# quartiq/stabilizer-stream

Measured on NVIDIA B200. Metric: sustained MS/s through full PSD cascade, higher is better.
Workload: dtype f32

## Files before the change

### stabilizer_stream_b200/csrc/sspsd_cascade.cu

```cuda
#if defined(__x86_64__)
#include <emmintrin.h>
#endif

#include "sspsd_cascade.cuh"

#include <algorithm>
#include <cmath>
#include <cstdlib>
#include <cstring>
#include <mutex>

#include "sspsd_decim_kernel.cuh"
#include "sspsd_stage_kernel.cuh"
#include "sspsd_stage_kernel_r16.cuh"
#include "sspsd_stage_kernel_ring.cuh"
#include "sspsd_stage_kernel_w16.cuh"

namespace sspsd {

static thread_local std::string g_err;
void set_error(const std::string& msg) { g_err = msg; }
const char* last_error() { return g_err.c_str(); }

bool cuda_ok(cudaError_t e, const char* what)
// ... 78 lines not shown
        SSPSD_CUDA(cudaFuncSetAttribute(psd_stage_kernel_ring1x5, cudaFuncAttributeMaxDynamicSharedMemorySize,
                                        (int)stage_ring_smem_bytes(384, 1, 3, false)));
        return SSPSD_OK;
    }
    if (log2n == 9)
        SSPSD_CUDA(cudaFuncSetAttribute(psd_stage_kernel_w16, cudaFuncAttributeMaxDynamicSharedMemorySize,
                                        (int)stage_w16_smem_bytes(W16::MAX_T)));
    switch (log2n) {
#define X(L)                                                                   \
    case L:                                                                    \
        *nt = Plan<L>::NT;                                                     \
        return prepare_stage_t<L>(hop, Plan<L>::NT <= 256 ? 100 * 1024 : 200 * 1024, tmax);
        SSPSD_FOR_SIZES(X)
#undef X
    default:
        set_error("n_fft must be a power of two in 64..8192");
        return SSPSD_EINVAL;
    }
}

template <int MA, int MB, int MC, int PRESET>
int launch_decim_t(const DecimParams& p, int grid, cudaStream_t s)
{
    using GE = DecGeom<MA, MB, MC>;
    decim8_kernel<MA, MB, MC, PRESET><<<grid, DEC_NT, GE::SMEM_FLOATS * sizeof(float), s>>>(p);
    return cuda_ok(cudaGetLastError(), "decim8_kernel launch") ? SSPSD_OK : SSPSD_ECUDA;
}

template <int MA, int MB, int MC, int PRESET, int OB, int CTAS>
int launch_decim_tma_t(const DecimParams& p, long long n_out, int num_sms, cudaStream_t s)
{
    const int ntiles = (int)((n_out + OB - 1) / OB);
    const int grid = std::min(ntiles, num_sms * CTAS);
    decim8_tma_kernel<MA, MB, MC, PRESET, OB, CTAS><<<grid, DEC_NT, decim_tma_smem_bytes<MA, MB, MC, OB>(), s>>>(p, ntiles);
    return cuda_ok(cudaGetLastError(), "decim8_tma_kernel launch") ? SSPSD_OK : SSPSD_ECUDA;
}

template <int MA, int MB, int MC, int PRESET, int OB, int CTAS>
int launch_decim_async_t(const DecimParams& p, long long n_out, int num_sms, cudaStream_t s)
{
    const int ntiles = (int)((n_out + OB - 1) / OB);
    const int grid = std::min(ntiles, num_sms * CTAS);
    decim8_async_kernel<MA, MB, MC, PRESET, OB, CTAS><<<grid, DEC_NT, decim_async_smem_bytes<MA, MB, MC, OB>(), s>>>(p, ntiles);
    return cuda_ok(cudaGetLastError(), "decim8_async_kernel launch") ? SSPSD_OK : SSPSD_ECUDA;
}

template <int MA, int MB, int MC, int PRESET, int OB, int CTAS>
int launch_decim_pf_t(const DecimParams& p, long long n_out, int num_sms, cudaStream_t s)
{
    const int ntiles = (int)((n_out + OB - 1) / OB);
    const int grid = std::min(ntiles, num_sms * CTAS);
    decim8_pf_kernel<MA, MB, MC, PRESET, OB, CTAS><<<grid, DEC_NT, decim_pf_smem_bytes<MA, MB, MC, OB>(), s>>>(p, ntiles);
    return cuda_ok(cudaGetLastError(), "decim8_pf_kernel launch") ? SSPSD_OK : SSPSD_ECUDA;
}

int decim_halo(int preset)
{
    return preset == SSPSD_HBF_98 ? DecGeom<3, 6, 15>::HALO : DecGeom<5, 10, 23>::HALO;
}

int upload_taps_once(int device)
{
    static std::mutex mu;
    static bool done[64] = {false};
    std::lock_guard<std::mutex> lock(mu);
    if (device < 64 && done[device])
        return SSPSD_OK;
    static_assert(sizeof(sspsd_hbf_taps) == sizeof(float) * SSPSD_HBF_NPRESET * 3 * SSPSD_HBF_MAXTAPS, "tap table");
    {
        float t0[SSPSD_HBF_NPRESET][3][SSPSD_HBF_MAXTAPS + 1], t1[SSPSD_HBF_NPRESET][3][SSPSD_HBF_MAXTAPS + 1];
        for (int p = 0; p < SSPSD_HBF_NPRESET; ++p)
            for (int s = 0; s < 3; ++s)
                for (int i = 0; i <= SSPSD_HBF_MAXTAPS; ++i) {
                    t0[p][s][i] = i < SSPSD_HBF_MAXTAPS ? sspsd_hbf_taps[p][s][i] : 0.f;
                    t1[p][s][i] = i + 1 < SSPSD_HBF_MAXTAPS ? sspsd_hbf_taps[p][s][i + 1] : 0.f;
                }
        SSPSD_CUDA(cudaMemcpyToSymbol(c_hbf_taps, t0, sizeof(t0)));
        SSPSD_CUDA(cudaMemcpyToSymbol(c_hbf_taps_sh, t1, sizeof(t1)));
    }
    SSPSD_CUDA(cudaFuncSetAttribute(decim8_kernel<5, 10, 23, SSPSD_HBF_140>, cudaFuncAttributeMaxDynamicSharedMemorySize,
                                    (int)(DecGeom<5, 10, 23>::SMEM_FLOATS * sizeof(float))));
    SSPSD_CUDA(cudaFuncSetAttribute(decim8_kernel<3, 6, 15, SSPSD_HBF_98>, cudaFuncAttributeMaxDynamicSharedMemorySize,
                                    (int)(DecGeom<3, 6, 15>::SMEM_FLOATS * sizeof(float))));
    SSPSD_CUDA(cudaFuncSetAttribute(decim8_async_kernel<5, 10, 23, SSPSD_HBF_140, 960, 2>,
                                    cudaFuncAttributeMaxDynamicSharedMemorySize, (int)decim_async_smem_bytes<5, 10, 23, 960>()));
    SSPSD_CUDA(cudaFuncSetAttribute(decim8_async_kernel<5, 10, 23, SSPSD_HBF_140, 640, 3>,
                                    cudaFuncAttributeMaxDynamicSharedMemorySize, (int)decim_async_smem_bytes<5, 10, 23, 640>()));
    SSPSD_CUDA(cudaFuncSetAttribute(decim8_async_kernel<3, 6, 15, SSPSD_HBF_98, 960, 2>,
                                    cudaFuncAttributeMaxDynamicSharedMemorySize, (int)decim_async_smem_bytes<3, 6, 15, 960>()));
    SSPSD_CUDA(cudaFuncSetAttribute(decim8_async_kernel<3, 6, 15, SSPSD_HBF_98, 640, 3>,
                                    cudaFuncAttributeMaxDynamicSharedMemorySize, (int)decim_async_smem_bytes<3, 6, 15, 640>()));
    SSPSD_CUDA(cudaFuncSetAttribute(decim8_tma_kernel<5, 10, 23, SSPSD_HBF_140, 960, 2>,
                                    cudaFuncAttributeMaxDynamicSharedMemorySize, (int)decim_tma_smem_bytes<5, 10, 23, 960>()));
    SSPSD_CUDA(cudaFuncSetAttribute(decim8_tma_kernel<5, 10, 23, SSPSD_HBF_140, 640, 3>,
                                    cudaFuncAttributeMaxDynamicSharedMemorySize, (int)decim_tma_smem_bytes<5, 10, 23, 640>()));
    SSPSD_CUDA(cudaFuncSetAttribute(decim8_tma_kernel<3, 6, 15, SSPSD_HBF_98, 960, 2>,
                                    cudaFuncAttributeMaxDynamicSharedMemorySize, (int)decim_tma_smem_bytes<3, 6, 15, 960>()));
    SSPSD_CUDA(cudaFuncSetAttribute(decim8_tma_kernel<3, 6, 15, SSPSD_HBF_98, 640, 3>,
                                    cudaFuncAttributeMaxDynamicSharedMemorySize, (int)decim_tma_smem_bytes<3, 6, 15, 640>()));
    SSPSD_CUDA(cudaFuncSetAttribute(decim8_tma_kernel<5, 10, 23, SSPSD_HBF_140, 768, 3>,
                                    cudaFuncAttributeMaxDynamicSharedMemorySize, (int)decim_tma_smem_bytes<5, 10, 23, 768>()));
    SSPSD_CUDA(cudaFuncSetAttribute(decim8_tma_kernel<3, 6, 15, SSPSD_HBF_98, 768, 3>,
                                    cudaFuncAttributeMaxDynamicSharedMemorySize, (int)decim_tma_smem_bytes<3, 6, 15, 768>()));
    SSPSD_CUDA(cudaFuncSetAttribute(decim8_pf_kernel<5, 10, 23, SSPSD_HBF_140, 960, 2>,
                                    cudaFuncAttributeMaxDynamicSharedMemorySize, (int)decim_pf_smem_bytes<5, 10, 23, 960>()));
    SSPSD_CUDA(cudaFuncSetAttribute(decim8_pf_kernel<5, 10, 23, SSPSD_HBF_140, 640, 3>,
                                    cudaFuncAttributeMaxDynamicSharedMemorySize, (int)decim_pf_smem_bytes<5, 10, 23, 640>()));
    SSPSD_CUDA(cudaFuncSetAttribute(decim8_pf_kernel<3, 6, 15, SSPSD_HBF_98, 960, 2>,
                                    cudaFuncAttributeMaxDynamicSharedMemorySize, (int)decim_pf_smem_bytes<3, 6, 15, 960>()));
    SSPSD_CUDA(cudaFuncSetAttribute(decim8_pf_kernel<3, 6, 15, SSPSD_HBF_98, 640, 3>,
                                    cudaFuncAttributeMaxDynamicSharedMemorySize, (int)decim_pf_smem_bytes<3, 6, 15, 640>()));
    if (device < 64)
        done[device] = true;
    return SSPSD_OK;
}

EwmaPlan ewma_plan(uint32_t count, uint32_t avg, uint64_t S)
{
    EwmaPlan e{};
    uint32_t steady = avg + 1u;
    e.g_s = (float)avg / (float)steady;
    uint64_t jb;
    if (count > avg) {
        jb = 0;
        e.g_first = (float)avg / (float)count;
    } else {
        jb = (uint64_t)avg - count + 1;
        e.g_first = e.g_s;
    }
    if (jb >= S) {
        e.jb = (int)S;
        e.total = 1.0f;
        e.count_after = (uint32_t)(count + S);
    } else {
        e.jb = (int)jb;
        double t = (double)e.g_first;
        uint64_t n_s = S - 1 - jb;
        if (n_s > 0)
            t *= std::pow((double)e.g_s, (double)n_s);
        e.total = (float)t;
        e.count_after = steady;
    }
    return e;
}

}

int hbf_info(int hbf, uint32_t* drain, uint32_t* halo)
{
    if (hbf != SSPSD_HBF_98 && hbf != SSPSD_HBF_140) return SSPSD_EINVAL;
    if (drain) *drain = (uint32_t)sspsd_hbf_drain[hbf];
    if (halo) *halo = (uint32_t)decim_halo(hbf);
    return SSPSD_OK;
}

Cascade::~Cascade()
{
    if (n_ == 0)
        return;
    DeviceGuard g(cfg_.device);
    if (stream_)
        cudaStreamSynchronize(stream_);
    if (deep_stream_) cudaStreamSynchronize(deep_stream_);
    if (psd_stream_) cudaStreamSynchronize(psd_stream_);
// ... 65 lines not shown
    std::vector<float> win(n);
    if (cfg.window == SSPSD_WINDOW_RECT) {
        std::fill(win.begin(), win.end(), 1.0f);
        win_ = {1.0f, 1.0f, 0};
    } else {
        const float pi = 3.14159265358979323846f;
        float df = pi / (float)n;
        for (uint32_t i = 0; i < n; ++i) {
            float s = sinf(df * (float)i);
            win[i] = s * s;
        }
        win_ = {0.25f, 1.5f, n / 2};
    }
    hop_ = n - win_.overlap;
    drain_ = sspsd_hbf_drain[cfg.hbf];
    int halo = decim_halo(cfg.hbf);
    hb_ = std::max<int>((int)win_.overlap, halo);
    hb_ = (hb_ + 7) & ~7;

    SSPSD_CUDA(cudaDeviceGetAttribute(&num_sms_, cudaDevAttrMultiProcessorCount, cfg.device));
    if (cfg.stream) {
        stream_ = (cudaStream_t)cfg.stream;
    } else {
        SSPSD_CUDA(cudaStreamCreateWithFlags(&stream_, cudaStreamNonBlocking));
        own_stream_ = true;
    }
    SSPSD_CUDA(cudaStreamCreateWithFlags(&copy_stream_, cudaStreamNonBlocking));
    const char* ov = getenv("SSPSD_OVERLAP");
    deep_from_ = ov ? (size_t)atoi(ov) : 1;
    if (max_stages_ > 1 && deep_from_ > 0 && !one_stream_) {
        int lo_prio = 0, hi_prio = 0;
        SSPSD_CUDA(cudaDeviceGetStreamPriorityRange(&lo_prio, &hi_prio));
        SSPSD_CUDA(cudaStreamCreateWithPriority(&deep_stream_, cudaStreamNonBlocking, hi_prio));
        SSPSD_CUDA(cudaEventCreateWithFlags(&ev_stage0_, cudaEventDisableTiming));
        SSPSD_CUDA(cudaEventCreateWithFlags(&ev_deep_, cudaEventDisableTiming));
        const char* ps = getenv("SSPSD_PSD_STREAM");
        if (!ps || atoi(ps) != 0) {
            SSPSD_CUDA(cudaStreamCreateWithPriority(&psd_stream_, cudaStreamNonBlocking, hi_prio));
            SSPSD_CUDA(cudaEventCreateWithFlags(&ev_psd_join_, cudaEventDisableTiming));
        }
    }
    for (int i = 0; i < 2; ++i) {
        SSPSD_CUDA(cudaEventCreateWithFlags(&ev_copied_[i], cudaEventDisableTiming));
        SSPSD_CUDA(cudaEventCreateWithFlags(&ev_free_[i], cudaEventDisableTiming));
        SSPSD_CUDA(cudaEventCreateWithFlags(&ev_stage_[i], cudaEventDisableTiming));
    }
    int rc = upload_taps_once(cfg.device);
    if (rc) return rc;
    defer_ = cfg_.deep_defer ? cfg_.deep_defer : (1ull << 26);
    if (const char* e = getenv("SSPSD_DEFER")) defer_ = strtoull(e, nullptr, 0);
    k2_variant_ = k2_variant_from_env();
    {
        const char* e = getenv("SSPSD_K3");
        std::string m = e ? e : "tma960";
        k3_variant_ = m == "tiled" ? 0 : m == "tma960" ? 1 : m == "tma640" ? 2 : m == "async640" ? 4 : m == "pf960" ? 5 :
                      m == "pf640" ? 6 : m == "tma768" ? 7 : 3;
    }
    rc = prepare_stage((int)log2n_, k2_variant_ >= 1, (int)hop_, &tmax_, &nt_);
    if (rc) return rc;

    const uint32_t m = n / 2;
    std::vector<float2> twM(m), twN(m);
    for (uint32_t k = 0; k < m; ++k) {
        double a = -2.0 * M_PI * (double)k / (double)m;
        twM[k] = make_float2((float)std::cos(a), (float)std::sin(a));
        double b = -2.0 * M_PI * (double)k / (double)n;
        twN[k] = make_float2((float)std::cos(b), (float)std::sin(b));
    }
    acc_stride_ = (m + 1 + 63) & ~63u;
    SSPSD_CUDA(cudaMalloc(&d_win_, n * sizeof(float)));
    SSPSD_CUDA(cudaMalloc(&d_twM_, m * sizeof(float2)));
    SSPSD_CUDA(cudaMalloc(&d_twN_, m * sizeof(float2)));
    SSPSD_CUDA(cudaMalloc(&d_acc_, (size_t)SSPSD_MAX_STAGES * acc_stride_ * sizeof(float)));
    SSPSD_CUDA(cudaMemcpyAsync(d_win_, win.data(), n * sizeof(float), cudaMemcpyHostToDevice, stream_));
    SSPSD_CUDA(cudaMemcpyAsync(d_twM_, twM.data(), m * sizeof(float2), cudaMemcpyHostToDevice, stream_));
    SSPSD_CUDA(cudaMemcpyAsync(d_twN_, twN.data(), m * sizeof(float2), cudaMemcpyHostToDevice, stream_));
    SSPSD_CUDA(cudaMemsetAsync(d_acc_, 0, (size_t)SSPSD_MAX_STAGES * acc_stride_ * sizeof(float), stream_));
    SSPSD_CUDA(cudaMallocHost(&h_acc_, (size_t)SSPSD_MAX_STAGES * acc_stride_ * sizeof(float)));
    SSPSD_CUDA(cudaStreamSynchronize(stream_));
    stages_.reserve(SSPSD_MAX_STAGES);
    n_ = n;
    return SSPSD_OK;
}

uint32_t Cascade::stage_avg(size_t i) const
{
    unsigned sh = (unsigned)(SSPSD_DEPTH * i);
    uint32_t v = sh >= 32 ? 0u : (avg_.count >> sh);
    return std::min(v, avg_.limit);
}

int Cascade::add_stage()
{
    if (stages_.size() >= SSPSD_MAX_STAGES) {
        set_error("too many stages");
        return SSPSD_EINVAL;
    }
    StageState st;
    const size_t cap = (size_t)hb_ + n_ + 16;
    cudaStream_t ss = stage_stream(stages_.size());
    if (!spare_.empty()) {
        StageState old = spare_.back();
        spare_.pop_back();
        st.carry[0] = old.carry[0];
        st.carry[1] = old.carry[1];
        st.fresh[0] = old.fresh[0];
        st.fresh[1] = old.fresh[1];
        st.fresh_cap = old.fresh_cap;
        st.ev_read[0] = old.ev_read[0];
// ... 156 lines not shown
    rc = launch_stage((int)log2n_, k2_variant_ >= 1, p, grid, psd_stream(i));
    prof_end(psd_stream(i));
    if (rc) return rc;
    return reduce_partials(i, grid * groups, p);
}

int Cascade::prepare_partials(size_t i, int rows, StageParams* p)
{
    p->part = nullptr;
    p->part_stride = 0;
    if (!(cfg_.flags & SSPSD_FLAG_DETERMINISTIC)) return SSPSD_OK;
    const int which = psd_stream(i) == stream_ ? 0 : 1;
    const size_t need = (size_t)rows * acc_stride_;
    if (need > part_cap_[which]) {
        SSPSD_CUDA(cudaStreamSynchronize(psd_stream(i)));
        if (d_part_[which]) SSPSD_CUDA(cudaFree(d_part_[which]));
        d_part_[which] = nullptr;
        SSPSD_CUDA(cudaMalloc(&d_part_[which], need * sizeof(float)));
        part_cap_[which] = need;
    }
    p->part = d_part_[which];
    p->part_stride = (int)acc_stride_;
    return SSPSD_OK;
}

int Cascade::reduce_partials(size_t i, int rows, const StageParams& p)
{
    if (!p.part) return SSPSD_OK;
    const int nb = (int)(n_ / 2 + 1);
    prof_begin(SSPSD_PROF_OTHER, 0, psd_stream(i));
    reduce_partials_kernel<<<(nb + 127) / 128, 128, 0, psd_stream(i)>>>(p.acc, p.part, rows, p.part_stride, nb);
    prof_end(psd_stream(i));
    return cuda_ok(cudaGetLastError(), "reduce_partials_kernel launch") ? SSPSD_OK : SSPSD_ECUDA;
}

int Cascade::launch_decim(size_t i, const StreamSrc& src, uint64_t m0, uint64_t m1, float* out_fresh,
                          long long out_split, long long out_cap)
{
    DecimParams p{};
    p.src = src;
    p.m0 = (long long)m0;
    p.m1 = (long long)m1;
    p.drain = drain_;
    p.out_fresh = out_fresh;
    p.out_split = out_split;
    p.out_cap = out_cap;
    p.preset = cfg_.hbf;
    long long lo = std::max<long long>(p.m0, p.drain);
    if (p.m1 <= lo)
        return SSPSD_OK;
    int grid = (int)((p.m1 - lo + DEC_OB - 1) / DEC_OB);
    cudaStream_t ss = stage_stream(i);
    static const bool fuse_carry = !getenv("SSPSD_CARRY_KERNEL");
    if (cc_valid_ && fuse_carry && (k3_variant_ == 1 || k3_variant_ == 2 || k3_variant_ == 7)) {
        p.cc = cc_pending_;
        cc_valid_ = false;
    }
    prof_begin(i == 0 ? SSPSD_PROF_DECIM_STAGE0 : SSPSD_PROF_DECIM_DEEP, (uint64_t)(p.m1 - lo) * 8, ss);
    int rc;
    if (k3_variant_ == 0) {
        rc = cfg_.hbf == SSPSD_HBF_98 ? launch_decim_t<3, 6, 15, SSPSD_HBF_98>(p, grid, ss)
                                      : launch_decim_t<5, 10, 23, SSPSD_HBF_140>(p, grid, ss);
    } else if (k3_variant_ == 1) {
        rc = cfg_.hbf == SSPSD_HBF_98 ? launch_decim_tma_t<3, 6, 15, SSPSD_HBF_98, 960, 2>(p, p.m1 - lo, num_sms_, ss)
                                      : launch_decim_tma_t<5, 10, 23, SSPSD_HBF_140, 960, 2>(p, p.m1 - lo, num_sms_, ss);
    } else if (k3_variant_ == 2) {
        rc = cfg_.hbf == SSPSD_HBF_98 ? launch_decim_tma_t<3, 6, 15, SSPSD_HBF_98, 640, 3>(p, p.m1 - lo, num_sms_, ss)
                                      : launch_decim_tma_t<5, 10, 23, SSPSD_HBF_140, 640, 3>(p, p.m1 - lo, num_sms_, ss);
    } else if (k3_variant_ == 3) {
        rc = cfg_.hbf == SSPSD_HBF_98 ? launch_decim_async_t<3, 6, 15, SSPSD_HBF_98, 960, 2>(p, p.m1 - lo, num_sms_, ss)
                                      : launch_decim_async_t<5, 10, 23, SSPSD_HBF_140, 960, 2>(p, p.m1 - lo, num_sms_, ss);
    } else if (k3_variant_ == 7) {
        rc = cfg_.hbf == SSPSD_HBF_98 ? launch_decim_tma_t<3, 6, 15, SSPSD_HBF_98, 768, 3>(p, p.m1 - lo, num_sms_, ss)
                                      : launch_decim_tma_t<5, 10, 23, SSPSD_HBF_140, 768, 3>(p, p.m1 - lo, num_sms_, ss);
    } else if (k3_variant_ == 5) {
        rc = cfg_.hbf == SSPSD_HBF_98 ? launch_decim_pf_t<3, 6, 15, SSPSD_HBF_98, 960, 2>(p, p.m1 - lo, num_sms_, ss)
                                      : launch_decim_pf_t<5, 10, 23, SSPSD_HBF_140, 960, 2>(p, p.m1 - lo, num_sms_, ss);
    } else if (k3_variant_ == 6) {
        rc = cfg_.hbf == SSPSD_HBF_98 ? launch_decim_pf_t<3, 6, 15, SSPSD_HBF_98, 640, 3>(p, p.m1 - lo, num_sms_, ss)
                                      : launch_decim_pf_t<5, 10, 23, SSPSD_HBF_140, 640, 3>(p, p.m1 - lo, num_sms_, ss);
    } else {
        rc = cfg_.hbf == SSPSD_HBF_98 ? launch_decim_async_t<3, 6, 15, SSPSD_HBF_98, 640, 3>(p, p.m1 - lo, num_sms_, ss)
                                      : launch_decim_async_t<5, 10, 23, SSPSD_HBF_140, 640, 3>(p, p.m1 - lo, num_sms_, ss);
    }
    prof_end(ss);
    return rc;
}

int Cascade::run_stage(size_t i, const float* fresh, long long split, uint64_t n_new)
{
    StageState& st = stages_[i];
    cudaStream_t ss = stage_stream(i);
    cudaStream_t ps = psd_stream(i);
    const uint64_t L1 = st.L + n_new;
    const uint64_t craw0 = st.craw;
    const uint64_t craw1 = L1 < n_ ? 0 : 1 + (L1 - n_) / hop_;
    const StreamSrc src{st.carry[st.cur], fresh, st.carry_start, split, (long long)L1};
    int rc;
    bool psd_launched = false;
    if (ps != ss && craw1 > craw0) {
        SSPSD_CUDA(cudaEventRecord(st.ev_in, ss));
        SSPSD_CUDA(cudaStreamWaitEvent(ps, st.ev_in, 0));
    }

    if (windowed_ && i < n_local_ && craw1 > craw0) {
        const uint64_t step = (uint64_t)hop_ << (SSPSD_DEPTH * i);
        const uint64_t c = own_offset(i);
        auto first_at_or_after = [&](uint64_t pos) { return pos <= c ? 0ull : (pos - c + step - 1) / step; };
        uint64_t klo = std::max<uint64_t>(first_at_or_after(own_lo_), (st.valid_from + hop_ - 1) / hop_);
        uint64_t khi = own_hi_ == ~0ull ? ~0ull : first_at_or_after(own_hi_);
        uint64_t a = std::max(craw0, klo), b = std::min(craw1, khi);
        if (b > a) {
            if (st.avg == 0xffffffffu) {
// ... 943 lines not shown
```

### stabilizer_stream_b200/csrc/sspsd_cascade.cuh

```cuda
#pragma once
#include <cuda_runtime.h>

#include <cstdint>
#include <string>
#include <vector>

#include "../../include/sspsd.h"
#include "sspsd_device.cuh"

namespace sspsd {

struct StageParams;
void set_error(const std::string& msg);
const char* last_error();
int hbf_info(int hbf, uint32_t* drain, uint32_t* halo);
bool cuda_ok(cudaError_t e, const char* what);

struct DeviceGuard {
    int prev = -1;
    bool ok = true;
    explicit DeviceGuard(int dev)
    {
        if (cudaGetDevice(&prev) != cudaSuccess) prev = -1;
        ok = prev == dev || cuda_ok(cudaSetDevice(dev), "cudaSetDevice");
// ... 105 lines not shown
    cudaStream_t stage_stream(size_t i) const { return (i < deep_from_ || !deep_stream_) ? stream_ : deep_stream_; }
    cudaStream_t psd_stream(size_t i) const { return (i >= deep_from_ && psd_stream_) ? psd_stream_ : stage_stream(i); }
    int join_streams();
    uint64_t defer_threshold(size_t j) const;
    int run_pending(size_t j);
    int flush_deferred();
    int ensure_fresh(StageState& st, size_t need, size_t reserve = 0);
    int ensure_in_buffers(size_t need);
    int process_host(const float* x, size_t n);
    int flush_staged();
    int feed_device_chunk(const float* x, size_t n);
    int feed_host_chunk(const float* xh, size_t n);
    static uint64_t host_chunk() { return 1ull << 23; }
    float gain_of(uint32_t count) const;
    uint32_t stage_avg(size_t i) const;
    uint64_t decimated(const StageState& st) const { return st.craw ? n_ + (st.craw - 1) * (uint64_t)hop_ : 0; }

    struct ProfRec {
        int cls;
        cudaEvent_t a, b;
        uint64_t units;
    };
    bool prof_on_ = false;
    std::vector<ProfRec> prof_;
    uint64_t launches_[SSPSD_PROF_NCLASS] = {0, 0, 0, 0, 0};
    void prof_begin(int cls, uint64_t units, cudaStream_t s);
    void prof_end(cudaStream_t s);

    bool windowed_ = false;
    uint64_t own_lo_ = 0, own_hi_ = ~0ull;
    uint32_t n_local_ = SSPSD_MAX_STAGES;
    float* d_tail_ = nullptr;
    size_t tail_cap_ = 0, tail_len_ = 0;
    uint64_t tail_first_ = 0;
    uint64_t seek_pos_ = 0;
    uint64_t next_valid_from(uint64_t valid) const;
    uint64_t own_offset(size_t i) const;

    StageHook* hook_ = nullptr;
    bool one_stream_ = false;
    sspsd_config cfg_{};
    uint32_t n_ = 0, log2n_ = 0, hop_ = 0, max_stages_ = SSPSD_MAX_STAGES;
    WindowInfo win_{};
    int detrend_ = 0;
    sspsd_avg_opts avg_{0xffffffffu, 0xffffffffu};
    int hb_ = 0;
    int drain_ = 0;
    int num_sms_ = 148;
    int tmax_ = 1, nt_ = 256;
    uint64_t defer_ = 1ull << 26;
    uint64_t defer_window_ = 0;
    CarryJob cc_pending_{};
    bool cc_valid_ = false;
    int k3_variant_ = 1;
    int k2_variant_ = 2;
    bool single_stage_avg_set_ = false;
    uint32_t single_stage_avg_ = 0xffffffffu;
    cudaStream_t stream_ = nullptr;
    bool own_stream_ = false;
    cudaStream_t copy_stream_ = nullptr;
    cudaStream_t deep_stream_ = nullptr;
    cudaStream_t psd_stream_ = nullptr;
    cudaEvent_t ev_stage0_ = nullptr, ev_deep_ = nullptr, ev_psd_join_ = nullptr;
    bool deep_dirty_ = false, psd_dirty_ = false;
    size_t deep_from_ = 1;
    cudaEvent_t ev_copied_[2] = {nullptr, nullptr}, ev_free_[2] = {nullptr, nullptr};
    cudaEvent_t ev_stage_[2] = {nullptr, nullptr};
    int last_copy_ = -1;
    std::vector<StageState> stages_;
    std::vector<StageState> spare_;
    float* d_win_ = nullptr;
    float2* d_twM_ = nullptr;
    float2* d_twN_ = nullptr;
    float* d_acc_ = nullptr;
    uint32_t acc_stride_ = 0;
    float* h_stage_[2] = {nullptr, nullptr};
    int stage_buf_ = 0;
    bool stage_pending_[2] = {false, false};
    size_t staged_ = 0;
    float* d_in_[2] = {nullptr, nullptr};
    size_t d_in_cap_ = 0;
    int in_buf_ = 0;
    float* h_acc_ = nullptr;
    float* d_part_[2] = {nullptr, nullptr};
    size_t part_cap_[2] = {0, 0};
    float* d_sink_ = nullptr;
    size_t sink_cap_ = 0, sink_len_ = 0;
};

}

struct sspsd_cascade {
    sspsd::Cascade c;
};
struct sspsd_stage {
    sspsd::Cascade c;
};
```

### stabilizer_stream_b200/csrc/sspsd_decim_kernel.cuh

```cuda
#pragma once
#include "sspsd_device.cuh"
#include "sspsd_hbf_taps.h"

namespace sspsd {

__constant__ __align__(8) float c_hbf_taps[SSPSD_HBF_NPRESET][3][SSPSD_HBF_MAXTAPS + 1];
__constant__ __align__(8) float c_hbf_taps_sh[SSPSD_HBF_NPRESET][3][SSPSD_HBF_MAXTAPS + 1];

constexpr int DEC_OB = 960;
constexpr int DEC_P = 8;
constexpr int DEC_LP = 3;
constexpr int DEC_NT = 256;

constexpr int roundup(int v, int m) { return (v + m - 1) / m * m; }

template <int MA, int MB, int MC, int OB_ = DEC_OB>
struct DecGeom {
    static constexpr int OB = OB_;
    static constexpr int NB = roundup(2 * OB + 4 * MC - 2, DEC_P);
    static constexpr int NA = roundup(2 * NB + 4 * MB - 2, DEC_P);
    static constexpr int NX = roundup(2 * NA + 4 * MA - 2, 8);
    static constexpr int HALO = NX - 8 * OB;
    static constexpr int phase_stride(int len) { return ((len + DEC_P - 1) / DEC_P + 27) / 32 * 32 + 4; }
    static constexpr int SX = phase_stride(NX / 2), SA = phase_stride(NA / 2), SB = phase_stride(NB / 2);
    static constexpr int SMEM_FLOATS = 2 * DEC_P * (SX + SA + SB);
};

__device__ __forceinline__ void carry_job(const StreamSrc& src, const CarryJob& c)
{
    SSPSD_ASSERT(c.n >= 0 && c.n <= c.dst_cap && c.head_n >= 0 && c.head_n < 4);
    for (int i = blockIdx.x * blockDim.x + threadIdx.x; i < c.n; i += gridDim.x * blockDim.x) {
        const float v = ld_stream1(src, c.g0 + i);
        c.dst[i] = v;
        if (i >= c.n - c.head_n) c.head_dst[i - (c.n - c.head_n)] = v;
    }
}

struct DecimParams {
    CarryJob cc;
    StreamSrc src;
    long long m0, m1;
    long long drain;
    float* out_fresh;
    long long out_split;
    long long out_cap;
    int preset;
};

template <int M, int SI, int SO, int REL0, bool FINAL, int PRESET, int SET>
__device__ __forceinline__ void hbf_stage(const float* __restrict__ ine, const float* __restrict__ ino,
                                          int n_out, float* __restrict__ oute,
                                          float* __restrict__ outo, float* __restrict__ gout, int rel_lo, int rel_hi,
                                          long long gidx0 = 0, long long gcap = 0)
{
    (void)gidx0;
    (void)gcap;
    constexpr int P = DEC_P, LP = DEC_LP;
    for (int w = threadIdx.x; w < n_out / P; w += DEC_NT) {
        constexpr int NW = 2 * M + P - 1;
        float2 wp[(NW + 1) / 2];
#pragma unroll
        for (int i = 0; i < NW; ++i) {
            const int c = REL0 - 2 * M + 1 + i;
            const float x = ino[(c & (P - 1)) * SI + (c >> LP) + w];
            if (i & 1) wp[i >> 1].y = x; else wp[i >> 1].x = x;
        }
        const float2* __restrict__ tp0 = reinterpret_cast<const float2*>(&c_hbf_taps[PRESET][SET][0]);
        const float2* __restrict__ tp1 = reinterpret_cast<const float2*>(&c_hbf_taps_sh[PRESET][SET][0]);
        float y[P];
#pragma unroll
        for (int q = 0; q < P; ++q) {
            float2 acc = make_float2(0.f, 0.f);
            constexpr int dummy = 0;
            (void)dummy;
            const int i0 = q & 1;
#pragma unroll
            for (int i = i0; i + 1 < M; i += 2) {
                const float2 l = wp[(q + i) >> 1];
                const float2 r = wp[(q + 2 * M - 2 - i) >> 1];
                const float2 sum = __fadd2_rn(l, make_float2(r.y, r.x));
                acc = __ffma2_rn(sum, (q & 1) ? tp1[(i - 1) >> 1] : tp0[i >> 1], acc);
            }
            float a = acc.x + acc.y;
            auto winv = [&](int k) { return (k & 1) ? wp[k >> 1].y : wp[k >> 1].x; };
            if (q & 1) a = fmaf(winv(q) + winv(q + 2 * M - 1), c_hbf_taps[PRESET][SET][0], a);
            if (((M - i0) & 1) != 0) a = fmaf(winv(q + M - 1) + winv(q + M), c_hbf_taps[PRESET][SET][M - 1], a);
            const int ce = REL0 + q - M + 1;
            y[q] = ine[(ce & (P - 1)) * SI + (ce >> LP) + w] + a;
        }
        if constexpr (FINAL) {
#pragma unroll
            for (int q = 0; q < P; ++q) {
                const int r = P * w + q;
                if (r >= rel_lo && r < rel_hi) {
                    SSPSD_ASSERT(gidx0 + r >= 0 && gidx0 + r < gcap);
                    gout[r] = y[q];
                }
            }
        } else {
            const int pb = (w & 1) * (P / 2) * SO + (w >> 1);
#pragma unroll
            for (int r = 0; r < P / 2; ++r) {
                oute[pb + r * SO] = y[2 * r];
                outo[pb + r * SO] = y[2 * r + 1];
            }
        }
    }
}

template <int MA, int MB, int MC, int PRESET>
__global__ void __launch_bounds__(DEC_NT) decim8_kernel(const DecimParams p)
{
    using GE = DecGeom<MA, MB, MC>;
    extern __shared__ __align__(16) float smem[];
    float* xe = smem;
    float* xo = xe + DEC_P * GE::SX;
    float* ae = xo + DEC_P * GE::SX;
    float* ao = ae + DEC_P * GE::SA;
    float* be = ao + DEC_P * GE::SA;
    float* bo = be + DEC_P * GE::SB;

    const long long mhi = p.m1 - (long long)blockIdx.x * DEC_OB;
    const long long x_base = 8 * mhi - GE::NX;
    const long long c_base = mhi - DEC_OB;

    if (x_base >= p.src.split) {
        const float4* __restrict__ gx = reinterpret_cast<const float4*>(p.src.fresh + (x_base - p.src.split));
        constexpr int NV = GE::NX / 4;
#pragma unroll 2
        for (int v0 = 0; v0 < NV; v0 += 4 * DEC_NT) {
            float4 f[4];
#pragma unroll
            for (int u = 0; u < 4; ++u) {
                const int v = v0 + u * DEC_NT + threadIdx.x;
                if (v < NV) f[u] = __ldg(gx + v);
            }
#pragma unroll
            for (int u = 0; u < 4; ++u) {
                const int v = v0 + u * DEC_NT + threadIdx.x;
                if (v < NV) {
                    const int pos = 2 * (v & 3) * GE::SX + (v >> 2);
// ... 194 lines not shown
            if (v < NV) {
                const int pos = 2 * (v & 3) * GE::SX + (v >> 2);
                xe[pos] = pf[u].x;
                xo[pos] = pf[u].y;
                xe[pos + GE::SX] = pf[u].z;
                xo[pos + GE::SX] = pf[u].w;
            }
        }
    };
    int tile = blockIdx.x;
    if (tile < ntiles) {
        fetch(tile);
        scatter();
    }
    const long long lo = p.m0 > p.drain ? p.m0 : p.drain;
    for (; tile < ntiles; tile += gridDim.x) {
        const long long mhi = p.m1 - (long long)tile * OB;
        const long long c_base = mhi - OB;
        const int next = tile + (int)gridDim.x;
        __syncthreads();
        if (next < ntiles) fetch(next);
        hbf_stage<MA, GE::SX, GE::SA, GE::NX / 2 - GE::NA, false, PRESET, 2>(xe, xo, GE::NA, ae, ao, nullptr, 0, 0);
        __syncthreads();
        hbf_stage<MB, GE::SA, GE::SB, GE::NA / 2 - GE::NB, false, PRESET, 1>(ae, ao, GE::NB, be, bo, nullptr, 0, 0);
        __syncthreads();
        if (next < ntiles) scatter();
        const int rel_lo = lo > c_base ? (int)(lo - c_base) : 0;
        hbf_stage<MC, GE::SB, GE::SB, GE::NB / 2 - OB, true, PRESET, 0>(be, bo, OB, nullptr, nullptr,
                                                                        p.out_fresh + (c_base - p.drain - p.out_split),
                                                                        rel_lo, OB, c_base - p.drain - p.out_split, p.out_cap);
    }
}

template <int MA, int MB, int MC, int OB>
constexpr size_t decim_pf_smem_bytes()
{
    return (size_t)DecGeom<MA, MB, MC, OB>::SMEM_FLOATS * sizeof(float);
}

template <int MA, int MB, int MC, int OB>
constexpr size_t decim_async_smem_bytes()
{
    using GE = DecGeom<MA, MB, MC, OB>;
    return (size_t)(2 * (2 * DEC_P * GE::SX + 4) + 2 * DEC_P * (GE::SA + GE::SB)) * sizeof(float);
}

template <int MA, int MB, int MC, int OB>
constexpr size_t decim_tma_smem_bytes()
{
    using GE = DecGeom<MA, MB, MC, OB>;
    return (size_t)(GE::NX + GE::SMEM_FLOATS) * sizeof(float) + 16;
}

__global__ void carry_copy_kernel(StreamSrc src, long long g0, int n, float* __restrict__ dst,
                                  float* __restrict__ head_dst, int head_n, int dst_cap)
{
    carry_job(src, CarryJob{g0, n, head_n, dst, head_dst, dst_cap});
}

}
```

Before: 240,700.

## Add swizzled 2D TMA decimator kernel with register-window first stage as default

Adds a new decimation kernel that loads input as 32-float rows through a 2D tensor map with 128B swizzle, double-buffered via mbarriers. The first half-band stage reads each thread's row from shared memory into registers and computes 16 outputs per thread, optionally fetching halo values through warp shuffles, before feeding stages B and C. Phase blocking of 8 or 16 is selectable, and the new variant becomes the default K3 path with carry fusion enabled. This is meant to cut shared-memory bank conflicts and the deinterleave cost of the input stage. The cost is a host-side tensor map encode on every launch and a 96-float register array that raises register pressure.

After: 245,500, median of 6. About the same (+2.0%).

```diff
diff --git a/stabilizer_stream_b200/csrc/sspsd_cascade.cu b/stabilizer_stream_b200/csrc/sspsd_cascade.cu
--- a/stabilizer_stream_b200/csrc/sspsd_cascade.cu
+++ b/stabilizer_stream_b200/csrc/sspsd_cascade.cu
@@ -154,6 +154,58 @@
     const int grid = std::min(ntiles, num_sms * CTAS);
     decim8_pf_kernel<MA, MB, MC, PRESET, OB, CTAS><<<grid, DEC_NT, decim_pf_smem_bytes<MA, MB, MC, OB>(), s>>>(p, ntiles);
     return cuda_ok(cudaGetLastError(), "decim8_pf_kernel launch") ? SSPSD_OK : SSPSD_ECUDA;
+}
+
+using TensorMapEncodeTiled = CUresult (*)(CUtensorMap*, CUtensorMapDataType, cuuint32_t, void*, const cuuint64_t*,
+                                          const cuuint64_t*, const cuuint32_t*, const cuuint32_t*, CUtensorMapInterleave,
+                                          CUtensorMapSwizzle, CUtensorMapL2promotion, CUtensorMapFloatOOBfill);
+static TensorMapEncodeTiled tensor_map_encoder()
+{
+    static const TensorMapEncodeTiled f = [] {
+        void* fn = nullptr;
+        cudaDriverEntryPointQueryResult q{};
+        if (cudaGetDriverEntryPoint("cuTensorMapEncodeTiled", &fn, cudaEnableDefault, &q) != cudaSuccess ||
+            q != cudaDriverEntryPointSuccess)
+            fn = nullptr;
+        return reinterpret_cast<TensorMapEncodeTiled>(fn);
+    }();
+    return f;
+}
+
+template <int MA, int MB, int MC, int PRESET, int OB, int CTAS, int PBC, bool HSHFL>
+int launch_decim_swz_t(const DecimParams& p, long long n_out, int num_sms, cudaStream_t s)
+{
+    using GE = DecGeom<MA, MB, MC, OB>;
+    using SG = SwzGeom<MA, MB, MC, OB, PBC>;
+    const int ntiles = (int)((n_out + OB - 1) / OB);
+    const int grid = std::min(ntiles, num_sms * CTAS);
+    const long long r0 = 8 * p.m1 - GE::NX + SG::ROW0;
+    const long long g0 = p.src.split + (((r0 - p.src.split) % 32) + 32) % 32;
+    const long long rows = p.src.end > g0 ? std::min<long long>((p.src.end - g0) / 32, 1ll << 30) : 0;
+    alignas(64) CUtensorMap map;
+    std::memset(&map, 0, sizeof(map));
+    int tm_rows = 0;
+    if (rows >= SG::NR) {
+        const TensorMapEncodeTiled encode = tensor_map_encoder();
+        if (!encode) {
+            set_error("cuTensorMapEncodeTiled is not available from the CUDA driver");
+            return SSPSD_ECUDA;
+        }
+        const cuuint64_t dims[2] = {32, (cuuint64_t)rows};
+        const cuuint64_t strides[1] = {32 * sizeof(float)};
+        const cuuint32_t box[2] = {32, (cuuint32_t)SG::NR};
+        const cuuint32_t estr[2] = {1, 1};
+        const CUresult r = encode(&map, CU_TENSOR_MAP_DATA_TYPE_FLOAT32, 2, const_cast<float*>(p.src.fresh + (g0 - p.src.split)),
+                                  dims, strides, box, estr, CU_TENSOR_MAP_INTERLEAVE_NONE, CU_TENSOR_MAP_SWIZZLE_128B,
+                                  CU_TENSOR_MAP_L2_PROMOTION_L2_256B, CU_TENSOR_MAP_FLOAT_OOB_FILL_NONE);
+        if (r != CUDA_SUCCESS) {
+            set_error("cuTensorMapEncodeTiled failed: " + std::to_string((int)r));
+            return SSPSD_ECUDA;
+        }
+        tm_rows = (int)rows;
+    }
+    decim8_swz_kernel<MA, MB, MC, PRESET, OB, CTAS, PBC, HSHFL><<<grid, DEC_NT, SG::SMEM_BYTES, s>>>(map, p, ntiles, g0, tm_rows);
+    return cuda_ok(cudaGetLastError(), "decim8_swz_kernel launch") ? SSPSD_OK : SSPSD_ECUDA;
 }
 
 int decim_halo(int preset)
@@ -212,6 +264,26 @@
                                     cudaFuncAttributeMaxDynamicSharedMemorySize, (int)decim_pf_smem_bytes<3, 6, 15, 960>()));
     SSPSD_CUDA(cudaFuncSetAttribute(decim8_pf_kernel<3, 6, 15, SSPSD_HBF_98, 640, 3>,
                                     cudaFuncAttributeMaxDynamicSharedMemorySize, (int)decim_pf_smem_bytes<3, 6, 15, 640>()));
+    SSPSD_CUDA(cudaFuncSetAttribute(decim8_swz_kernel<5, 10, 23, SSPSD_HBF_140, 960, 2, 8, false>, cudaFuncAttributeMaxDynamicSharedMemorySize,
+                                    (int)SwzGeom<5, 10, 23, 960, 8>::SMEM_BYTES));
+    SSPSD_CUDA(cudaFuncSetAttribute(decim8_swz_kernel<3, 6, 15, SSPSD_HBF_98, 960, 2, 8, false>, cudaFuncAttributeMaxDynamicSharedMemorySize,
+                                    (int)SwzGeom<3, 6, 15, 960, 8>::SMEM_BYTES));
+    SSPSD_CUDA(cudaFuncSetAttribute(decim8_swz_kernel<5, 10, 23, SSPSD_HBF_140, 960, 2, 16, false>, cudaFuncAttributeMaxDynamicSharedMemorySize,
+                                    (int)SwzGeom<5, 10, 23, 960, 16>::SMEM_BYTES));
+    SSPSD_CUDA(cudaFuncSetAttribute(decim8_swz_kernel<3, 6, 15, SSPSD_HBF_98, 960, 2, 16, false>, cudaFuncAttributeMaxDynamicSharedMemorySize,
+                                    (int)SwzGeom<3, 6, 15, 960, 16>::SMEM_BYTES));
+    SSPSD_CUDA(cudaFuncSetAttribute(decim8_swz_kernel<5, 10, 23, SSPSD_HBF_140, 960, 2, 8, true>, cudaFuncAttributeMaxDynamicSharedMemorySize,
+                                    (int)SwzGeom<5, 10, 23, 960, 8>::SMEM_BYTES));
+    SSPSD_CUDA(cudaFuncSetAttribute(decim8_swz_kernel<3, 6, 15, SSPSD_HBF_98, 960, 2, 8, true>, cudaFuncAttributeMaxDynamicSharedMemorySize,
+                                    (int)SwzGeom<3, 6, 15, 960, 8>::SMEM_BYTES));
+    SSPSD_CUDA(cudaFuncSetAttribute(decim8_swz_kernel<5, 10, 23, SSPSD_HBF_140, 640, 3, 8, false>, cudaFuncAttributeMaxDynamicSharedMemorySize,
+                                    (int)SwzGeom<5, 10, 23, 640, 8>::SMEM_BYTES));
+    SSPSD_CUDA(cudaFuncSetAttribute(decim8_swz_kernel<3, 6, 15, SSPSD_HBF_98, 640, 3, 8, false>, cudaFuncAttributeMaxDynamicSharedMemorySize,
+                                    (int)SwzGeom<3, 6, 15, 640, 8>::SMEM_BYTES));
+    SSPSD_CUDA(cudaFuncSetAttribute(decim8_swz_kernel<5, 10, 23, SSPSD_HBF_140, 640, 3, 8, true>, cudaFuncAttributeMaxDynamicSharedMemorySize,
+                                    (int)SwzGeom<5, 10, 23, 640, 8>::SMEM_BYTES));
+    SSPSD_CUDA(cudaFuncSetAttribute(decim8_swz_kernel<3, 6, 15, SSPSD_HBF_98, 640, 3, 8, true>, cudaFuncAttributeMaxDynamicSharedMemorySize,
+                                    (int)SwzGeom<3, 6, 15, 640, 8>::SMEM_BYTES));
     if (device < 64)
         done[device] = true;
     return SSPSD_OK;
@@ -383,9 +455,9 @@
     k2_variant_ = k2_variant_from_env();
     {
         const char* e = getenv("SSPSD_K3");
-        std::string m = e ? e : "tma960";
+        std::string m = e ? e : "swz960";
         k3_variant_ = m == "tiled" ? 0 : m == "tma960" ? 1 : m == "tma640" ? 2 : m == "async640" ? 4 : m == "pf960" ? 5 :
-                      m == "pf640" ? 6 : m == "tma768" ? 7 : 3;
+                      m == "pf640" ? 6 : m == "tma768" ? 7 : m == "swz960" ? 8 : m == "swz960w16" ? 9 : m == "swz960s" ? 10 : m == "swz640" ? 11 : m == "swz640s" ? 12 : 3;
     }
     rc = prepare_stage((int)log2n_, k2_variant_ >= 1, (int)hop_, &tmax_, &nt_);
     if (rc) return rc;
@@ -648,13 +720,30 @@
     int grid = (int)((p.m1 - lo + DEC_OB - 1) / DEC_OB);
     cudaStream_t ss = stage_stream(i);
     static const bool fuse_carry = !getenv("SSPSD_CARRY_KERNEL");
-    if (cc_valid_ && fuse_carry && (k3_variant_ == 1 || k3_variant_ == 2 || k3_variant_ == 7)) {
+    if (cc_valid_ && fuse_carry && (k3_variant_ == 1 || k3_variant_ == 2 || k3_variant_ >= 7)) {
         p.cc = cc_pending_;
         cc_valid_ = false;
     }
     prof_begin(i == 0 ? SSPSD_PROF_DECIM_STAGE0 : SSPSD_PROF_DECIM_DEEP, (uint64_t)(p.m1 - lo) * 8, ss);
     int rc;
-    if (k3_variant_ == 0) {
+    if (k3_variant_ >= 8) {
+        if (k3_variant_ == 8) {
+            rc = cfg_.hbf == SSPSD_HBF_98 ? launch_decim_swz_t<3, 6, 15, SSPSD_HBF_98, 960, 2, 8, false>(p, p.m1 - lo, num_sms_, ss)
+                                          : launch_decim_swz_t<5, 10, 23, SSPSD_HBF_140, 960, 2, 8, false>(p, p.m1 - lo, num_sms_, ss);
+        } else if (k3_variant_ == 9) {
+            rc = cfg_.hbf == SSPSD_HBF_98 ? launch_decim_swz_t<3, 6, 15, SSPSD_HBF_98, 960, 2, 16, false>(p, p.m1 - lo, num_sms_, ss)
+                                          : launch_decim_swz_t<5, 10, 23, SSPSD_HBF_140, 960, 2, 16, false>(p, p.m1 - lo, num_sms_, ss);
+        } else if (k3_variant_ == 10) {
+            rc = cfg_.hbf == SSPSD_HBF_98 ? launch_decim_swz_t<3, 6, 15, SSPSD_HBF_98, 960, 2, 8, true>(p, p.m1 - lo, num_sms_, ss)
+                                          : launch_decim_swz_t<5, 10, 23, SSPSD_HBF_140, 960, 2, 8, true>(p, p.m1 - lo, num_sms_, ss);
+        } else if (k3_variant_ == 11) {
+            rc = cfg_.hbf == SSPSD_HBF_98 ? launch_decim_swz_t<3, 6, 15, SSPSD_HBF_98, 640, 3, 8, false>(p, p.m1 - lo, num_sms_, ss)
+                                          : launch_decim_swz_t<5, 10, 23, SSPSD_HBF_140, 640, 3, 8, false>(p, p.m1 - lo, num_sms_, ss);
+        } else if (k3_variant_ == 12) {
+            rc = cfg_.hbf == SSPSD_HBF_98 ? launch_decim_swz_t<3, 6, 15, SSPSD_HBF_98, 640, 3, 8, true>(p, p.m1 - lo, num_sms_, ss)
+                                          : launch_decim_swz_t<5, 10, 23, SSPSD_HBF_140, 640, 3, 8, true>(p, p.m1 - lo, num_sms_, ss);
+        }
+    } else if (k3_variant_ == 0) {
         rc = cfg_.hbf == SSPSD_HBF_98 ? launch_decim_t<3, 6, 15, SSPSD_HBF_98>(p, grid, ss)
                                       : launch_decim_t<5, 10, 23, SSPSD_HBF_140>(p, grid, ss);
     } else if (k3_variant_ == 1) {
diff --git a/stabilizer_stream_b200/csrc/sspsd_cascade.cuh b/stabilizer_stream_b200/csrc/sspsd_cascade.cuh
--- a/stabilizer_stream_b200/csrc/sspsd_cascade.cuh
+++ b/stabilizer_stream_b200/csrc/sspsd_cascade.cuh
@@ -181,7 +181,7 @@
     uint64_t defer_window_ = 0;
     CarryJob cc_pending_{};
     bool cc_valid_ = false;
-    int k3_variant_ = 1;
+    int k3_variant_ = 8;
     int k2_variant_ = 2;
     bool single_stage_avg_set_ = false;
     uint32_t single_stage_avg_ = 0xffffffffu;
diff --git a/stabilizer_stream_b200/csrc/sspsd_decim_kernel.cuh b/stabilizer_stream_b200/csrc/sspsd_decim_kernel.cuh
--- a/stabilizer_stream_b200/csrc/sspsd_decim_kernel.cuh
+++ b/stabilizer_stream_b200/csrc/sspsd_decim_kernel.cuh
@@ -1,4 +1,6 @@
 #pragma once
+#include <cuda.h>
+
 #include "sspsd_device.cuh"
 #include "sspsd_hbf_taps.h"
 
@@ -9,7 +11,6 @@
 
 constexpr int DEC_OB = 960;
 constexpr int DEC_P = 8;
-constexpr int DEC_LP = 3;
 constexpr int DEC_NT = 256;
 
 constexpr int roundup(int v, int m) { return (v + m - 1) / m * m; }
@@ -47,7 +48,28 @@
     int preset;
 };
 
-template <int M, int SI, int SO, int REL0, bool FINAL, int PRESET, int SET>
+template <int M, int PRESET, int SET, int NWP>
+__device__ __forceinline__ float hbf_out(const float2 (&wp)[NWP], int q, float centre)
+{
+    const float2* __restrict__ tp0 = reinterpret_cast<const float2*>(&c_hbf_taps[PRESET][SET][0]);
+    const float2* __restrict__ tp1 = reinterpret_cast<const float2*>(&c_hbf_taps_sh[PRESET][SET][0]);
+    float2 acc = make_float2(0.f, 0.f);
+    const int i0 = q & 1;
+#pragma unroll
+    for (int i = i0; i + 1 < M; i += 2) {
+        const float2 l = wp[(q + i) >> 1];
+        const float2 r = wp[(q + 2 * M - 2 - i) >> 1];
+        const float2 sum = __fadd2_rn(l, make_float2(r.y, r.x));
+        acc = __ffma2_rn(sum, (q & 1) ? tp1[(i - 1) >> 1] : tp0[i >> 1], acc);
+    }
+    float a = acc.x + acc.y;
+    auto winv = [&](int k) { return (k & 1) ? wp[k >> 1].y : wp[k >> 1].x; };
+    if (q & 1) a = fmaf(winv(q) + winv(q + 2 * M - 1), c_hbf_taps[PRESET][SET][0], a);
+    if (((M - i0) & 1) != 0) a = fmaf(winv(q + M - 1) + winv(q + M), c_hbf_taps[PRESET][SET][M - 1], a);
+    return centre + a;
+}
+
+template <int M, int SI, int SO, int REL0, bool FINAL, int PRESET, int SET, int P = DEC_P>
 __device__ __forceinline__ void hbf_stage(const float* __restrict__ ine, const float* __restrict__ ino,
                                           int n_out, float* __restrict__ oute,
                                           float* __restrict__ outo, float* __restrict__ gout, int rel_lo, int rel_hi,
@@ -55,7 +77,8 @@
 {
     (void)gidx0;
     (void)gcap;
-    constexpr int P = DEC_P, LP = DEC_LP;
+    static_assert(P == 8 || P == 16, "outputs per thread");
+    constexpr int LP = P == 8 ? 3 : 4;
     for (int w = threadIdx.x; w < n_out / P; w += DEC_NT) {
         constexpr int NW = 2 * M + P - 1;
         float2 wp[(NW + 1) / 2];
@@ -65,28 +88,11 @@
             const float x = ino[(c & (P - 1)) * SI + (c >> LP) + w];
             if (i & 1) wp[i >> 1].y = x; else wp[i >> 1].x = x;
         }
-        const float2* __restrict__ tp0 = reinterpret_cast<const float2*>(&c_hbf_taps[PRESET][SET][0]);
-        const float2* __restrict__ tp1 = reinterpret_cast<const float2*>(&c_hbf_taps_sh[PRESET][SET][0]);
         float y[P];
 #pragma unroll
         for (int q = 0; q < P; ++q) {
-            float2 acc = make_float2(0.f, 0.f);
-            constexpr int dummy = 0;
-            (void)dummy;
-            const int i0 = q & 1;
-#pragma unroll
-            for (int i = i0; i + 1 < M; i += 2) {
-                const float2 l = wp[(q + i) >> 1];
-                const float2 r = wp[(q + 2 * M - 2 - i) >> 1];
-                const float2 sum = __fadd2_rn(l, make_float2(r.y, r.x));
-                acc = __ffma2_rn(sum, (q & 1) ? tp1[(i - 1) >> 1] : tp0[i >> 1], acc);
-            }
-            float a = acc.x + acc.y;
-            auto winv = [&](int k) { return (k & 1) ? wp[k >> 1].y : wp[k >> 1].x; };
-            if (q & 1) a = fmaf(winv(q) + winv(q + 2 * M - 1), c_hbf_taps[PRESET][SET][0], a);
-            if (((M - i0) & 1) != 0) a = fmaf(winv(q + M - 1) + winv(q + M), c_hbf_taps[PRESET][SET][M - 1], a);
             const int ce = REL0 + q - M + 1;
-            y[q] = ine[(ce & (P - 1)) * SI + (ce >> LP) + w] + a;
+            y[q] = hbf_out<M, PRESET, SET>(wp, q, ine[(ce & (P - 1)) * SI + (ce >> LP) + w]);
         }
         if constexpr (FINAL) {
 #pragma unroll
@@ -387,6 +393,163 @@
     return (size_t)(GE::NX + GE::SMEM_FLOATS) * sizeof(float) + 16;
 }
 
+template <int MA, int MB, int MC, int OB, int PBC>
+struct SwzGeom {
+    using GE = DecGeom<MA, MB, MC, OB>;
+    static constexpr int REL0A = GE::NX / 2 - GE::NA;
+    static constexpr int RHO = 2 * (REL0A - MA + 1);
+    static constexpr int ROW0 = RHO - 32;
+    static constexpr int KA = (GE::NA + 15) / 16;
+    static constexpr int NR = (GE::NX - ROW0 + 31) / 32;
+    static constexpr int CLO = (32 - (2 * MA - 1)) / 4;
+    static constexpr int CHI = (2 * MA - 3) / 4;
+    static constexpr int STG = 32 * roundup(NR, 8);
+    static constexpr int pstride(int len)
+    {
+        return PBC == 8 ? GE::phase_stride(len) : ((len + 15) / 16 + 1) / 4 * 4 + 2;
+    }
+    static constexpr int SA = pstride(8 * KA), SB = pstride(GE::NB / 2);
+    static constexpr size_t SMEM_BYTES = 1024 + (size_t)(2 * STG + 2 * PBC * (SA + SB)) * sizeof(float) + 16;
+    static_assert(RHO >= 0 && RHO < 32 && (RHO & 3) == 0, "row phase");
+    static_assert(NR <= 256 && KA <= DEC_NT && 2 * MA - 1 <= 32, "tile rows");
+    static_assert((8 * OB) % 32 == 0, "every tile of a launch has the same row phase");
+    static_assert(GE::NB % PBC == 0 && OB % PBC == 0, "stages B and C: whole blocks");
+};
+
+__device__ __forceinline__ void tma_load_2d(void* dst, const CUtensorMap* map, int c0, int c1, uint64_t* bar)
+{
+    asm volatile(
+        "cp.async.bulk.tensor.2d.shared::cluster.global.mbarrier::complete_tx::bytes [%0], [%1, {%2, %3}], [%4];" ::"r"(
+            smem_u32(dst)),
+        "l"(reinterpret_cast<uint64_t>(map)), "r"(c0), "r"(c1), "r"(smem_u32(bar))
+        : "memory");
+}
+
+template <int MA, int MB, int MC, int PRESET, int OB, int CTAS, int PBC, bool HSHFL>
+__global__ void __launch_bounds__(DEC_NT, CTAS)
+    decim8_swz_kernel(const __grid_constant__ CUtensorMap tmap, const DecimParams p, const int ntiles, const long long tm_g0,
+                      const int tm_rows)
+{
+    using GE = DecGeom<MA, MB, MC, OB>;
+    using SG = SwzGeom<MA, MB, MC, OB, PBC>;
+    constexpr int LPBC = PBC == 8 ? 3 : 4;
+    extern __shared__ __align__(16) unsigned char smem_raw[];
+    float* stg = reinterpret_cast<float*>(smem_raw + ((1024u - (smem_u32(smem_raw) & 1023u)) & 1023u));
+    float* ae = stg + 2 * SG::STG;
+    float* ao = ae + PBC * SG::SA;
+    float* be = ao + PBC * SG::SA;
+    float* bo = be + PBC * SG::SB;
+    uint64_t* bar = reinterpret_cast<uint64_t*>(bo + PBC * SG::SB);
+
+    const int tid = threadIdx.x;
+    if (tid == 0) {
+        mbar_init(bar, 1);
+        mbar_init(bar + 1, 1);
+        asm volatile("fence.mbarrier_init.release.cluster;" ::: "memory");
+    }
+    __syncthreads();
+    auto row0 = [&](int t) { return 8 * (p.m1 - (long long)t * OB) - GE::NX + SG::ROW0; };
+    auto by_tma = [&](int t) {
+        const long long g = row0(t);
+        return g >= tm_g0 && (g - tm_g0) / 32 + SG::NR <= tm_rows;
+    };
+    auto issue = [&](int t, int b) {
+        const long long g = row0(t);
+        const int row = (int)((g - tm_g0) >> 5);
+        SSPSD_ASSERT(((g - tm_g0) & 31) == 0 && row >= 0 && row + SG::NR <= tm_rows && g >= p.src.split &&
+                     g + 32ll * SG::NR <= p.src.end);
+        asm volatile("fence.proxy.async.shared::cta;" ::: "memory");
+        mbar_expect_tx(bar + b, SG::NR * 128u);
+        tma_load_2d(stg + b * SG::STG, &tmap, 0, row, bar + b);
+    };
+    auto fill = [&](int t, float* dst) {
+        const long long g = row0(t);
+        for (int v = tid; v < SG::NR * 8; v += DEC_NT) {
+            const int r = v >> 3, c = v & 7;
+            const long long gv = g + 4ll * v;
+            const float4 f = gv + 4 <= p.src.end ? ld_stream4(p.src, gv) : make_float4(0.f, 0.f, 0.f, 0.f);
+            *reinterpret_cast<float4*>(dst + 32 * r + 4 * (c ^ (r & 7))) = f;
+        }
+    };
+
+    int tile = blockIdx.x;
+    if (tid == 0 && tile < ntiles && by_tma(tile)) issue(tile, 0);
+    if (p.cc.n) carry_job(p.src, p.cc);
+    const long long lo = p.m0 > p.drain ? p.m0 : p.drain;
+    uint32_t phase = 0;
+    for (unsigned it = 0; tile < ntiles; tile += gridDim.x, ++it) {
+        const int b = (int)(it & 1u);
+        const float* sb = stg + b * SG::STG;
+        const int next = tile + (int)gridDim.x;
+        if (tid == 0 && next < ntiles && by_tma(next)) issue(next, b ^ 1);
+        if (by_tma(tile)) {
+            mbar_wait(bar + b, (phase >> b) & 1u);
+            phase ^= 1u << b;
+        } else {
+            fill(tile, stg + b * SG::STG);
+            __syncthreads();
+        }
+        if (HSHFL || tid < SG::KA) {
+            const int R = HSHFL ? min(tid + 1, SG::NR - 1) : tid + 1;
+            float xr[96];
+            auto chunk = [&](int r, int c, int at) {
+                asm volatile("ld.volatile.shared.v4.f32 {%0, %1, %2, %3}, [%4];"
+                             : "=f"(xr[at]), "=f"(xr[at + 1]), "=f"(xr[at + 2]), "=f"(xr[at + 3])
+                             : "r"(smem_u32(sb + 32 * r + 4 * (c ^ (r & 7)))));
+            };
+#pragma unroll
+            for (int c = 0; c < 8; ++c) chunk(R, c, 32 + 4 * c);
+            const int Rh = R + 1 < SG::NR ? R + 1 : SG::NR - 1;
+            if constexpr (HSHFL) {
+                const int lane = tid & 31;
+#pragma unroll
+                for (int j = 33 - 2 * MA; j < 32; j += 2) xr[j] = __shfl_up_sync(0xffffffffu, xr[j + 32], 1);
+#pragma unroll
+                for (int j = 65; j < 62 + 2 * MA; j += 2) xr[j] = __shfl_down_sync(0xffffffffu, xr[j - 32], 1);
+                if (lane == 0) {
+#pragma unroll
+                    for (int c = SG::CLO; c < 8; ++c) chunk(R - 1, c, 4 * c);
+                }
+                if (lane == 31) {
+#pragma unroll
+                    for (int c = 0; c <= SG::CHI; ++c) chunk(Rh, c, 64 + 4 * c);
+                }
+            } else {
+#pragma unroll
+                for (int c = SG::CLO; c < 8; ++c) chunk(R - 1, c, 4 * c);
+#pragma unroll
+                for (int c = 0; c <= SG::CHI; ++c) chunk(Rh, c, 64 + 4 * c);
+            }
+            constexpr int NW = 2 * MA + 15;
+            float2 wp[(NW + 1) / 2];
+#pragma unroll
+            for (int i = 0; i < NW; ++i) {
+                const float x = xr[32 + 2 * i + 1 - 2 * MA];
+                if (i & 1) wp[i >> 1].y = x; else wp[i >> 1].x = x;
+            }
+            float y[16];
+#pragma unroll
+            for (int q = 0; q < 16; ++q) y[q] = hbf_out<MA, PRESET, 2>(wp, q, xr[32 + 2 * q]);
+#pragma unroll
+            for (int r = 0; r < 8 && tid < SG::KA; ++r) {
+                const int i = 8 * tid + r;
+                const int pos = (i & (PBC - 1)) * SG::SA + (i >> LPBC);
+                ae[pos] = y[2 * r];
+                ao[pos] = y[2 * r + 1];
+            }
+        }
+        __syncthreads();
+        hbf_stage<MB, SG::SA, SG::SB, GE::NA / 2 - GE::NB, false, PRESET, 1, PBC>(ae, ao, GE::NB, be, bo, nullptr, 0, 0);
+        __syncthreads();
+        const long long mhi = p.m1 - (long long)tile * OB;
+        const long long c_base = mhi - OB;
+        const int rel_lo = lo > c_base ? (int)(lo - c_base) : 0;
+        hbf_stage<MC, SG::SB, SG::SB, GE::NB / 2 - OB, true, PRESET, 0, PBC>(be, bo, OB, nullptr, nullptr,
+                                                                             p.out_fresh + (c_base - p.drain - p.out_split),
+                                                                             rel_lo, OB, c_base - p.drain - p.out_split, p.out_cap);
+    }
+}
+
 __global__ void carry_copy_kernel(StreamSrc src, long long g0, int n, float* __restrict__ dst,
                                   float* __restrict__ head_dst, int head_n, int dst_cap)
 {
```
